# bacpop/sparrowhawk

Hardware: AMD Instinct MI355X
Metric: Gbases/s assembled, k=31 150bp reads (higher is better)
Workload: dtype u64

## Files before the change

### sparrowhawk_amd/csrc/count_part.h

```cpp
#pragma once
#include <hip/hip_runtime.h>
#include <stdint.h>
#include <type_traits>
#include "kmer.h"

namespace shk {

static constexpr int PART_THREADS = 1024;
static constexpr int COUNT_THREADS = 1024;
static constexpr int PART_MAX_P = 16384;

struct PartParams {
    uint32_t P, G, slice_cap;
    int k, m;
    uint32_t max_n;
};

template <int RW> struct Rec { uint64_t w[RW]; };

__device__ __forceinline__ uint64_t sel4(uint32_t b, uint64_t t0, uint64_t t1, uint64_t t2, uint64_t t3) {
    uint64_t lo = (b & 1) ? t1 : t0;
    uint64_t hi = (b & 1) ? t3 : t2;
    return (b & 2) ? hi : lo;
}
// ... 532 lines not shown
    const uint32_t want = 2u * rows;
    return want <= 8u ? 8u : 1u << (32 - __clz((int)(want - 1u)));
}
struct EmitRanges {
    unsigned long long *tab_cursor = nullptr;
    unsigned long long *off = nullptr;
    uint32_t *msk = nullptr, *start = nullptr, *cnt = nullptr, *broken = nullptr;
};

template <int W, typename LT>
__device__ __forceinline__ void table_emit(KmerTable<W> &tb, CountCtlCore &ctl, unsigned long long mine, uint32_t threshold,
                                           unsigned long long *__restrict__ histo, KeyArr<W> out_keys,
                                           uint32_t *__restrict__ out_cnt, unsigned long long out_cap,
                                           unsigned long long *__restrict__ out_cursor, LT *list,
                                           uint32_t *hist_accum = nullptr ,
                                           uint32_t bias = 0 ,
                                           const EmitRanges &er = EmitRanges{}, uint32_t er_g = 0xFFFFFFFFu ) {
    constexpr uint32_t S = KmerTable<W>::S;
    const int lane = threadIdx.x & 63;
    for (int o = 32; o > 0; o >>= 1) mine += __shfl_down(mine, o);
    if (lane == 0 && mine) atomicAdd(&ctl.n_inst, mine);
    for (uint32_t s = threadIdx.x; s < S; s += COUNT_THREADS) {
        uint32_t c = tb.cnt[s];
        if (bias && c) { c = c > 0xFFFFFFFFu - bias ? 0xFFFFFFFFu : c + bias; tb.cnt[s] = c; }
        const unsigned long long m1 = __ballot(c == 1u);
        if (lane == 0 && m1) atomicAdd(&ctl.histo[0], (uint32_t)__popcll(m1));
        if (c > 1u) atomicAdd(&ctl.histo[c >= 500 ? 499 : c - 1], 1u);
        const bool e = c > threshold;
        const unsigned long long em = __ballot(e);
        if (!em) continue;
        uint32_t wb = 0;
        if (lane == 0) wb = atomicAdd(&ctl.n_emit, (uint32_t)__popcll(em));
        wb = __shfl(wb, 0);
        if (e) list[wb + (uint32_t)__popcll(em & ((1ull << lane) - 1ull))] = (LT)s;
    }
    __syncthreads();
    const uint32_t n_emit = ctl.n_emit;
    if (threadIdx.x == 0) {
        unsigned long long base = n_emit ? atomicAdd(out_cursor, (unsigned long long)n_emit) : 0ull;
        if (er.tab_cursor && er_g != 0xFFFFFFFFu) {
            const uint32_t sz = gp_table_size(n_emit);
            const unsigned long long tab_base = atomicAdd(er.tab_cursor, ((unsigned long long)n_emit << 32) | sz);
            er.off[er_g] = (uint32_t)tab_base; er.msk[er_g] = sz - 1u; er.start[er_g] = (uint32_t)base; er.cnt[er_g] = n_emit;
        }
        ctl.emit_base_lo = (uint32_t)base; ctl.emit_base_hi = (uint32_t)(base >> 32);
    }
    if (hist_accum) {
        for (uint32_t b = threadIdx.x; b < 500; b += COUNT_THREADS) hist_accum[b] += ctl.histo[b];
    } else {
        for (uint32_t b = threadIdx.x; b < 500; b += COUNT_THREADS)
            if (ctl.histo[b]) atomicAdd(&histo[b], (unsigned long long)ctl.histo[b]);
    }
    if (!n_emit) return;
    __syncthreads();
    const unsigned long long gbase = ((unsigned long long)ctl.emit_base_hi << 32) | ctl.emit_base_lo;
    for (uint32_t i = threadIdx.x; i < n_emit; i += COUNT_THREADS) {
        const uint32_t sl = list[i];
        const unsigned long long o = gbase + i;
        if (o < out_cap) {
            Kmer<W> x;
            if constexpr (W == 1) x.w[0] = tb.key0[sl];
            else {
#pragma unroll
                for (int j = 0; j < W; j++) x.w[j] = tb.key[j][sl];
            }
            out_keys.store(o, x);
            out_cnt[o] = tb.cnt[sl];
        }
    }
}

struct OvfRec { uint32_t p, est_distinct; unsigned long long instances; };
struct OvfItem { uint32_t p, F, cap, pad; unsigned long long base; };
static constexpr uint32_t OVF_MAX_F = 256;

struct RunView {
    const unsigned long long *run_addr16;
    const uint32_t *run_cnt;
    uint32_t S;
    int k;
    const uint32_t *weights = nullptr;
    unsigned long long rec_base16 = 0;
};

__global__ __launch_bounds__(256) void k_make_runs(const uint32_t *__restrict__ fill, PartParams pp,
                                                   const uint64_t *recs, uint32_t rec_words,
                                                   unsigned long long *__restrict__ run_addr16,
                                                   uint32_t *__restrict__ run_cnt) {
    const uint64_t n = (uint64_t)pp.P * pp.G;
    const unsigned long long base16 = (unsigned long long)recs >> 4;
    for (uint64_t i = (uint64_t)blockIdx.x * blockDim.x + threadIdx.x; i < n; i += (uint64_t)gridDim.x * blockDim.x) {
        run_addr16[i] = base16 + i * pp.slice_cap * (rec_words / 2u);
        run_cnt[i] = min(fill[i], pp.slice_cap);
    }
}

__global__ __launch_bounds__(256) void k_part_totals(const uint32_t *__restrict__ fill, PartParams pp,
                                                     unsigned long long *__restrict__ totals) {
    const uint32_t p = blockIdx.x;
    unsigned long long t = 0;
    for (uint32_t g = threadIdx.x; g < pp.G; g += blockDim.x) t += min(fill[(uint64_t)p * pp.G + g], pp.slice_cap);
    for (int o = 32; o > 0; o >>= 1) t += __shfl_down(t, o);
    __shared__ unsigned long long part[4];
    if ((threadIdx.x & 63) == 0) part[threadIdx.x >> 6] = t;
    __syncthreads();
    if (threadIdx.x == 0) totals[p] = part[0] + part[1] + part[2] + part[3];
}

template <int RW>
__global__ __launch_bounds__(256) void k_pack_partition(const uint64_t *__restrict__ recs,
                                                        const uint32_t *__restrict__ fill, PartParams pp,
                                                        const unsigned long long *__restrict__ base,
                                                        uint64_t *__restrict__ dst) {
    __shared__ uint32_t pre[257];
    const uint32_t p = blockIdx.x;
    const int lane = threadIdx.x & 63;
    if (threadIdx.x < 64) {
        uint32_t run = 0;
        for (uint32_t g0 = 0; g0 < pp.G; g0 += 64) {
            const uint32_t g = g0 + threadIdx.x;
            const uint32_t f = g < pp.G ? min(fill[(uint64_t)p * pp.G + g], pp.slice_cap) : 0u;
            uint32_t incl = f;
            for (int o = 1; o < 64; o <<= 1) { uint32_t v = __shfl_up(incl, o); if (lane >= o) incl += v; }
            if (g < pp.G) pre[g] = run + incl - f;
            run += __shfl(incl, 63);
        }
        if (threadIdx.x == 0) pre[pp.G] = run;
    }
    __syncthreads();
    const uint32_t R = pre[pp.G];
    const uint64_t *src_p = recs + (uint64_t)p * pp.G * pp.slice_cap * RW;
    uint64_t *dst_p = dst + base[p] * RW;
    for (uint32_t r = threadIdx.x; r < R; r += blockDim.x) {
        uint32_t lo = 0, hi = pp.G;
        while (hi - lo > 1) { const uint32_t mid = (lo + hi) >> 1; if (pre[mid] <= r) lo = mid; else hi = mid; }
        const uint64_t *src = src_p + ((uint64_t)lo * pp.slice_cap + (r - pre[lo])) * RW;
#pragma unroll
        for (int o = 0; o < RW; o += 2)
            *reinterpret_cast<ulonglong2 *>(dst_p + (uint64_t)r * RW + o) = *reinterpret_cast<const ulonglong2 *>(src + o);
    }
}

template <int RW>
__global__ __launch_bounds__(256) void k_merge_runs(RunView rvw, const unsigned long long *__restrict__ base,
                                                    uint64_t *__restrict__ dst) {
    __shared__ uint32_t pre[257];
    __shared__ unsigned long long roff[256];
    const uint32_t p = blockIdx.x, S_runs = rvw.S;
    const int lane = threadIdx.x & 63;
    if (threadIdx.x < 64) {
        uint32_t run = 0;
        for (uint32_t g0 = 0; g0 < S_runs; g0 += 64) {
            const uint32_t g = g0 + threadIdx.x;
            const uint32_t f = g < S_runs ? rvw.run_cnt[(uint64_t)p * S_runs + g] : 0u;
            if (g < S_runs) roff[g] = rvw.run_addr16[(uint64_t)p * S_runs + g];
            uint32_t incl = f;
            for (int o = 1; o < 64; o <<= 1) { const uint32_t v = __shfl_up(incl, o); if (lane >= o) incl += v; }
            if (g < S_runs) pre[g] = run + incl - f;
            run += __shfl(incl, 63);
        }
        if (threadIdx.x == 0) pre[S_runs] = run;
    }
    __syncthreads();
    const uint32_t R = pre[S_runs];
    uint64_t *dst_p = dst + base[p] * RW;
    for (uint32_t r = threadIdx.x; r < R; r += blockDim.x) {
        uint32_t lo = 0, hi = S_runs;
        while (hi - lo > 1) { const uint32_t mid = (lo + hi) >> 1; if (pre[mid] <= r) lo = mid; else hi = mid; }
        const uint64_t *src = reinterpret_cast<const uint64_t *>(roff[lo] << 4) + (uint64_t)(r - pre[lo]) * RW;
#pragma unroll
        for (int o = 0; o < RW; o += 2)
            *reinterpret_cast<ulonglong2 *>(dst_p + (uint64_t)r * RW + o) = *reinterpret_cast<const ulonglong2 *>(src + o);
    }
}

template <int W, bool WEIGHTED = false >
__global__ __launch_bounds__(COUNT_THREADS) void k_count_partitions(
    RunView rvw, uint32_t n_parts, uint32_t threshold,
    unsigned long long *__restrict__ histo, KeyArr<W> out_keys, uint32_t *__restrict__ out_cnt,
    unsigned long long out_cap, unsigned long long *__restrict__ out_cursor,
    unsigned long long *__restrict__ n_inst, uint32_t *__restrict__ flags,
    const uint32_t *__restrict__ part_list ,
    OvfRec *__restrict__ ovf ,
    uint32_t *__restrict__ ovf_n,
    uint32_t *__restrict__ work_counter ,
    uint32_t probe_blocks, uint32_t defer_after ) {
    constexpr int RW = 2 * W;
    constexpr uint32_t S = CountShared<W>::S;
    __shared__ CountShared<W> tb;
    __shared__ CountCtl ctl;
    __shared__ uint32_t whist[500];
    __shared__ uint32_t wtot[4];
    const int lane = threadIdx.x & 63;
    const int k = rvw.k;
    const uint32_t S_runs = rvw.S;
    for (uint32_t b = threadIdx.x; b < 500; b += COUNT_THREADS) whist[b] = 0;
    if (threadIdx.x == 0) ctl.n_inst = 0;
    auto load_runs = [&](uint32_t pi, uint32_t &cnt, unsigned long long &addr) {
        cnt = 0; addr = 0;
        if (pi < n_parts && threadIdx.x < S_runs) {
            const uint32_t pp = part_list ? part_list[pi] : pi;
            cnt = rvw.run_cnt[(uint64_t)pp * S_runs + threadIdx.x];
            addr = rvw.run_addr16[(uint64_t)pp * S_runs + threadIdx.x];
        }
    };
    uint32_t nx_cnt; unsigned long long nx_addr;
    load_runs(blockIdx.x, nx_cnt, nx_addr);
  uint32_t pi_next = 0;
  for (uint32_t pi = blockIdx.x; pi < n_parts; pi = pi_next) {
    const uint32_t p = part_list ? part_list[pi] : pi;
    if (threadIdx.x == 0) ctl.next_pi = gridDim.x + atomicAdd(work_counter, 1u);
    {
        const uint32_t f = nx_cnt;
        uint32_t incl = f;
        if (threadIdx.x < 256) {
            for (int o = 1; o < 64; o <<= 1) { const uint32_t v = __shfl_up(incl, o); if (lane >= o) incl += v; }
            if (lane == 63) wtot[threadIdx.x >> 6] = incl;
        }
        __syncthreads();
        if (threadIdx.x < 256) {
            uint32_t off = 0;
            for (uint32_t w = 0; w < (threadIdx.x >> 6); w++) off += wtot[w];
            if (threadIdx.x < S_runs) { ctl.pre[threadIdx.x] = off + incl - f; ctl.roff[threadIdx.x] = nx_addr; }
        }
        if (threadIdx.x == 0) {
            ctl.pre[S_runs] = wtot[0] + wtot[1] + wtot[2] + wtot[3];
            ctl.sp = 1; ctl.st_res[0] = 0; ctl.st_step[0] = 1; ctl.st_factor[0] = 1; ctl.st_next[0] = 0;
            ctl.part_inst = 0; ctl.n_used = 0;
            uint32_t force = 0;
            if (ovf && defer_after && pi >= probe_blocks) {
                const uint32_t x = __hip_atomic_load(&ovf_n[1], __ATOMIC_RELAXED, __HIP_MEMORY_SCOPE_AGENT);
                const uint32_t n_over = x >> 16, n_tried = x & 0xFFFFu;
                force = (n_over >= defer_after && 4u * n_over >= 3u * n_tried) ? 1u : 0u;
            }
            ctl.overflow = force;
        }
    }
    __syncthreads();
    pi_next = ctl.next_pi;
    load_runs(pi_next, nx_cnt, nx_addr);
   [&]() {
    const uint32_t R = ctl.pre[S_runs];
    const bool sat = R >= (1u << 26) || WEIGHTED;

    auto defer = [&](unsigned long long mine, bool was_tried) {
        if (threadIdx.x == 0) ctl.tried = 0;
        __syncthreads();
        for (int o = 32; o > 0; o >>= 1) mine += __shfl_down(mine, o);
        if (lane == 0 && mine) atomicAdd(&ctl.tried, mine);
        unsigned long long inst = 0;
        for (uint32_t r = threadIdx.x; r < R; r += COUNT_THREADS) {
            uint32_t lo = 0, hi = S_runs;
            while (hi - lo > 1) { const uint32_t mid = (lo + hi) >> 1; if (ctl.pre[mid] <= r) lo = mid; else hi = mid; }
            const uint64_t *src = reinterpret_cast<const uint64_t *>(ctl.roff[lo] << 4) + (uint64_t)(r - ctl.pre[lo]) * RW;
            unsigned long long wgt = 1ull;
            if constexpr (WEIGHTED) wgt = rvw.weights[(ctl.roff[lo] - rvw.rec_base16) / W + (r - ctl.pre[lo])];
            inst += ((src[RW - 1] >> 58) + 1ull) * wgt;
        }
        for (int o = 32; o > 0; o >>= 1) inst += __shfl_down(inst, o);
        if (lane == 0 && inst) atomicAdd(&ctl.part_inst, inst);
        __syncthreads();
        if (threadIdx.x == 0 && R) {
            const double est = ctl.tried ? (double)ctl.n_used * (double)ctl.part_inst / (double)ctl.tried : (double)ctl.part_inst;
            const uint32_t slot = atomicAdd(ovf_n, 1u);
            OvfRec o; o.p = p; o.est_distinct = !was_tried ? 0u  : est > 4.0e9 ? 0xFFFFFFFFu : est < 1.0 ? 1u : (uint32_t)est; o.instances = ctl.part_inst;
            ovf[slot] = o;
        }
        if (threadIdx.x == 0 && was_tried && defer_after) atomicAdd(&ovf_n[1], 0x10001u);
    };
    if (ctl.overflow) { defer(0ull, false); return; }

    while (true) {
        __syncthreads();
        if (ctl.sp == 0) break;
        const uint32_t top = ctl.sp - 1;
        const uint32_t res = ctl.st_res[top] + ctl.st_next[top] * ctl.st_step[top], mod = ctl.st_step[top] * ctl.st_factor[top];
        __syncthreads();
        if (threadIdx.x == 0) {
            if (++ctl.st_next[top] == ctl.st_factor[top]) ctl.sp--;
            ctl.n_used = 0; ctl.overflow = 0; ctl.n_emit = 0; ctl.wave_cursor = 0; ctl.rec_used = 0;
            ctl.prog_num = 0; ctl.prog_den = 1;
        }
        table_reset<W>(tb, ctl);

        unsigned long long mine = 0;
        const uint32_t per_wave = (((R + (COUNT_THREADS / 64) - 1) / (COUNT_THREADS / 64)) + 63u) & ~63u;
        const uint32_t w_begin = min(R, (threadIdx.x >> 6) * per_wave), w_end = min(R, w_begin + per_wave);
        uint32_t run_lo = 0, run_next = 0;
        {
            uint32_t lo = 0, hi = S_runs;
            const uint32_t r = min(w_begin + (uint32_t)lane, R ? R - 1u : 0u);
            while (hi - lo > 1) { const uint32_t mid = (lo + hi) >> 1; if (ctl.pre[mid] <= r) lo = mid; else hi = mid; }
            run_lo = lo; run_next = ctl.pre[lo + 1];
        }
        auto fetch = [&](uint32_t r, Rec<RW> &rec, uint32_t &wgt) -> uint32_t {
            wgt = 1u;
            if (r >= w_end) return 0u;
            while (r >= run_next) { run_lo++; run_next = ctl.pre[run_lo + 1]; }
            const uint64_t *src = reinterpret_cast<const uint64_t *>(ctl.roff[run_lo] << 4) + (uint64_t)(r - ctl.pre[run_lo]) * RW;
            if constexpr (WEIGHTED) wgt = rvw.weights[(ctl.roff[run_lo] - rvw.rec_base16) / W + (r - ctl.pre[run_lo])];
#pragma unroll
            for (int o = 0; o < RW; o += 2) {
                const ulonglong2 v2 = *reinterpret_cast<const ulonglong2 *>(src + o);
                rec.w[o] = v2.x; rec.w[o + 1] = v2.y;
            }
            return 1u;
        };
        auto expand = [&](Rec<RW> rec, uint32_t n, uint32_t weight) {
            Kmer<W> f = km_zero<W>();
            for (uint32_t s = 0; s < n; s++) {
                if (ctl.overflow || ctl.n_used > (S / 10) * 9) return;
                if (s) {
#pragma unroll
                    for (int o = 0; o < RW - 1; o++) rec.w[o] = (rec.w[o] >> 2) | (rec.w[o + 1] << 62);
                    rec.w[RW - 1] >>= 2;
                }
                Kmer<W> rv;
#pragma unroll
                for (int j = 0; j < W; j++) rv.w[j] = ~rec.w[j];
                rv.w[W - 1] &= km_topmask<W>(k);
                if (s) km_push_back<W>(f, (uint32_t)(rec.w[W - 1] >> ((2 * (k - 1)) & 63)) & 3u, k);
                else f = km_revcomp<W>(rv, k);
                const bool use_r = km_less<W>(rv, f);
                Kmer<W> c;
#pragma unroll
                for (int j = 0; j < W; j++) c.w[j] = use_r ? rv.w[j] : f.w[j];
                const uint32_t h = km_mix32<W>(c);
                if (mod == 1 || ((h >> 20) & (mod - 1u)) == res) {
                    if (!lds_insert<W>(tb, ctl, c, h ^ __builtin_amdgcn_alignbit(h, h, 19), weight, sat)) ctl.overflow = 1;
                    mine += weight;
                }
            }
        };
        Rec<RW> nxt, nxt2;
#pragma unroll
        for (int o = 0; o < RW; o++) { nxt.w[o] = 0; nxt2.w[o] = 0; }
        uint32_t w_nxt, w_nxt2;
        uint32_t have_nxt = fetch(w_begin + (uint32_t)lane, nxt, w_nxt);
        uint32_t have_nxt2 = fetch(w_begin + 64u + (uint32_t)lane, nxt2, w_nxt2);
        if (threadIdx.x == 0) ctl.prog_den = R ? R : 1u;
        for (uint32_t r0 = w_begin; r0 < w_end; r0 += 64) {
            if (ctl.overflow || ctl.n_used > (S / 10) * 9) { atomicMax(&ctl.prog_num, min(R, (r0 - w_begin) * (COUNT_THREADS / 64) + 1u)); break; }
            Rec<RW> rec = nxt;
            const uint32_t n = have_nxt ? (uint32_t)(rec.w[RW - 1] >> 58) + 1u : 0u;
            if (n) rec_canonicalise<RW>(rec.w, n, k);
            const uint32_t wgt = w_nxt;
            nxt = nxt2; have_nxt = have_nxt2; w_nxt = w_nxt2;
            have_nxt2 = fetch(r0 + 128u + (uint32_t)lane, nxt2, w_nxt2);
            if (n && !rec_insert<W>(tb.rt, ctl, rec, wgt)) {
                if (ovf && mod == 1 && (r0 - w_begin) * 2u < (w_end - w_begin)) ctl.overflow = 1;
                else expand(rec, n, wgt);
            }
        }
        {
            constexpr uint32_t SRc = decltype(tb.rt)::SR;
            auto &rt = tb.rt;
            if (threadIdx.x < 64) rt.nhist[threadIdx.x] = 0;
            __syncthreads();
            for (uint32_t s = threadIdx.x; s < SRc; s += COUNT_THREADS)
                if (rt.rst[s] >= 3u) atomicAdd(&rt.nhist[(uint32_t)(rt.w[s][RW - 1] >> 58)], 1u);
            __syncthreads();
            if (threadIdx.x < 64) {
                const uint32_t v = rt.nhist[threadIdx.x];
                uint32_t incl = v;
                for (int o = 1; o < 64; o <<= 1) { const uint32_t u = __shfl_up(incl, o); if (lane >= o) incl += u; }
                rt.nbase[threadIdx.x] = incl - v;
                if (threadIdx.x == 63) ctl.n_recs = incl;
            }
            __syncthreads();
            for (uint32_t s = threadIdx.x; s < SRc; s += COUNT_THREADS)
                if (rt.rst[s] >= 3u) rt.order[atomicAdd(&rt.nbase[(uint32_t)(rt.w[s][RW - 1] >> 58)], 1u)] = (uint16_t)s;
            __syncthreads();
            const uint32_t n_recs = ctl.n_recs;
            if (threadIdx.x == 0 && ctl.prog_num == 0) ctl.prog_den = n_recs ? n_recs : 1u;
            __syncthreads();
            for (uint32_t i = threadIdx.x; i < n_recs; i += COUNT_THREADS) {
                if (ctl.overflow || ctl.n_used > (S / 10) * 9) { atomicMax(&ctl.prog_num, i - threadIdx.x + 1u); break; }
                const uint32_t s = rt.order[i];
                Rec<RW> rec;
#pragma unroll
                for (int o = 0; o < RW; o++) rec.w[o] = rt.w[s][o];
                expand(rec, (uint32_t)(rec.w[RW - 1] >> 58) + 1u, rt.rst[s] - 2u);
            }
        }
        __syncthreads();
        const bool over = ctl.overflow != 0 || ctl.n_used > (S / 10) * 9;
        if (over && ovf && mod == 1) {
            defer(mine, true);
            return;
        }
        if (over) {
            if (mod >= 4096 || ctl.sp + 1 > 16) { if (threadIdx.x == 0) flags[0] = 1; break; }
            __syncthreads();
            if (threadIdx.x == 0) {
                const uint32_t num = ctl.prog_num ? ctl.prog_num : ctl.prog_den;
                const double est = (double)ctl.n_used * (double)ctl.prog_den / (double)num;
                uint32_t factor = 2;
                while ((double)factor * (0.6 * S) < est && mod * factor < 4096u) factor <<= 1;
                ctl.st_res[ctl.sp] = res; ctl.st_step[ctl.sp] = mod; ctl.st_factor[ctl.sp] = factor; ctl.st_next[ctl.sp] = 0;
                ctl.sp += 1;
            }
            continue;
        }
        static_assert(2u * decltype(tb.rt)::SR >= S, "emit list");
        table_emit<W>(tb, ctl, mine, threshold, histo, out_keys, out_cnt, out_cap, out_cursor, reinterpret_cast<uint16_t *>(tb.rt.rst), whist);
    }
    if (threadIdx.x == 0 && ovf && defer_after) atomicAdd(&ovf_n[1], 1u);
   }();
  }
    __syncthreads();
    for (uint32_t b = threadIdx.x; b < 500; b += COUNT_THREADS)
        if (whist[b]) atomicAdd(&histo[b], (unsigned long long)whist[b]);
    if (threadIdx.x == 0 && ctl.n_inst) atomicAdd(n_inst, ctl.n_inst);
}


template <int W> struct DedupeShared {
    RecTable<W, (W == 1 ? 3072u : ((69632u / (16u * W + 6u)) & ~63u))> rt;
};
template <int W>
__global__ __launch_bounds__(COUNT_THREADS, W <= 2 ? 8 : 4) void k_dedupe_partitions(
                                                                     RunView rvw, uint32_t p_first, uint32_t n_parts,
                                                                     const unsigned long long *__restrict__ base ,
                                                                     unsigned long long base_stride,
                                                                     uint64_t *__restrict__ out_recs, uint32_t *__restrict__ out_w,
                                                                     uint32_t *__restrict__ n_out, uint32_t *__restrict__ work_counter,
                                                                     OvfRec *__restrict__ ovf , uint32_t *__restrict__ ovf_n,
                                                                     uint32_t defer_after, uint32_t kmer_cap,
                                                                     uint32_t *__restrict__ verdict_out ) {
    constexpr int RW = 2 * W;
    __shared__ DedupeShared<W> tb;
    __shared__ CountCtl ctl;
    __shared__ uint32_t wtot[4];
    constexpr uint32_t SR = decltype(tb.rt)::SR;
    const int lane = threadIdx.x & 63;
    const int k = rvw.k;
    const uint32_t S_runs = rvw.S;
    const uint32_t n_here = n_parts - p_first;
    __shared__ uint32_t forced_sh;
    if (threadIdx.x == 0) forced_sh = 0;
    __syncthreads();
    bool forced = false;
    uint32_t pi_next = 0;
    for (uint32_t pi = blockIdx.x; pi < n_here; pi = pi_next) {
        const uint32_t p = p_first + pi;
        uint32_t f = 0; unsigned long long addr = 0;
        if (threadIdx.x < S_runs) { f = rvw.run_cnt[(uint64_t)p * S_runs + threadIdx.x]; addr = rvw.run_addr16[(uint64_t)p * S_runs + threadIdx.x]; }
        forced = forced_sh != 0;
        if (forced) {
            unsigned long long inst = 0;
            const uint64_t *src = reinterpret_cast<const uint64_t *>(addr << 4);
            for (uint32_t i = 0; i < f; i++) inst += (src[(uint64_t)i * RW + RW - 1] >> 58) + 1ull;
            __syncthreads();
            if (threadIdx.x == 0) { ctl.part_inst = 0; ctl.next_pi = gridDim.x + atomicAdd(work_counter, 1u); }
            __syncthreads();
            for (int o = 32; o > 0; o >>= 1) inst += __shfl_down(inst, o);
            if (lane == 0 && inst) atomicAdd(&ctl.part_inst, inst);
            __syncthreads();
            pi_next = ctl.next_pi;
            if (threadIdx.x == 0) {
                n_out[p] = 0;
                if (ctl.part_inst) { const uint32_t slot = atomicAdd(ovf_n, 1u); OvfRec o; o.p = p; o.est_distinct = 0u; o.instances = ctl.part_inst; ovf[slot] = o; }
            }
            continue;
        }
        uint32_t incl = f;
        if (threadIdx.x < 256) {
            for (int o = 1; o < 64; o <<= 1) { const uint32_t v = __shfl_up(incl, o); if (lane >= o) incl += v; }
            if (lane == 63) wtot[threadIdx.x >> 6] = incl;
        }
        __syncthreads();
        if (threadIdx.x < 256) {
            uint32_t off = 0;
            for (uint32_t w = 0; w < (threadIdx.x >> 6); w++) off += wtot[w];
            if (threadIdx.x < S_runs) { ctl.pre[threadIdx.x] = off + incl - f; ctl.roff[threadIdx.x] = addr; }
        }
        if (threadIdx.x == 0) {
            ctl.pre[S_runs] = wtot[0] + wtot[1] + wtot[2] + wtot[3];
            ctl.rec_used = 0; ctl.n_emit = 0; ctl.part_inst = 0;
            ctl.next_pi = gridDim.x + atomicAdd(work_counter, 1u);
        }
        for (uint32_t s = threadIdx.x; s < SR; s += COUNT_THREADS) tb.rt.rst[s] = 0;
        __syncthreads();
        pi_next = ctl.next_pi;
        const uint32_t R = ctl.pre[S_runs];
        auto hand_over = [&]() {
            unsigned long long inst = 0;
            const uint32_t pw = (((R + (COUNT_THREADS / 64) - 1) / (COUNT_THREADS / 64)) + 63u) & ~63u;
            const uint32_t wb = min(R, (threadIdx.x >> 6) * pw), we = min(R, wb + pw);
            uint32_t lo = 0, hi = S_runs;
            { const uint32_t r = min(wb + (uint32_t)lane, R ? R - 1u : 0u);
              while (hi - lo > 1) { const uint32_t mid = (lo + hi) >> 1; if (ctl.pre[mid] <= r) lo = mid; else hi = mid; } }
            uint32_t nx = ctl.pre[lo + 1];
            for (uint32_t r = wb + (uint32_t)lane; r < we; r += 64) {
                while (r >= nx) { lo++; nx = ctl.pre[lo + 1]; }
                const uint64_t *src = reinterpret_cast<const uint64_t *>(ctl.roff[lo] << 4) + (uint64_t)(r - ctl.pre[lo]) * RW;
                inst += (src[RW - 1] >> 58) + 1ull;
            }
            for (int o = 32; o > 0; o >>= 1) inst += __shfl_down(inst, o);
            if (lane == 0 && inst) atomicAdd(&ctl.part_inst, inst);
            __syncthreads();
            if (threadIdx.x == 0) {
                n_out[p] = 0;
                if (R) { const uint32_t slot = atomicAdd(ovf_n, 1u); OvfRec o; o.p = p; o.est_distinct = 0u; o.instances = ctl.part_inst; ovf[slot] = o; }
            }
        };
        const unsigned long long base_p = base ? base[p] : (unsigned long long)p * base_stride;
        uint64_t *dst = out_recs + base_p * RW;
        uint32_t *dst_w = out_w + base_p;
        const uint32_t per_wave = (((R + (COUNT_THREADS / 64) - 1) / (COUNT_THREADS / 64)) + 63u) & ~63u;
        const uint32_t w_begin = min(R, (threadIdx.x >> 6) * per_wave), w_end = min(R, w_begin + per_wave);
        uint32_t run_lo = 0, run_next = 0;
        {
            uint32_t lo = 0, hi = S_runs;
            const uint32_t r = min(w_begin + (uint32_t)lane, R ? R - 1u : 0u);
            while (hi - lo > 1) { const uint32_t mid = (lo + hi) >> 1; if (ctl.pre[mid] <= r) lo = mid; else hi = mid; }
            run_lo = lo; run_next = ctl.pre[lo + 1];
        }
        auto fetch = [&](uint32_t r, Rec<RW> &rec) -> uint32_t {
            if (r >= w_end) return 0u;
            while (r >= run_next) { run_lo++; run_next = ctl.pre[run_lo + 1]; }
            const uint64_t *src = reinterpret_cast<const uint64_t *>(ctl.roff[run_lo] << 4) + (uint64_t)(r - ctl.pre[run_lo]) * RW;
#pragma unroll
            for (int o = 0; o < RW; o += 2) {
                const ulonglong2 v2 = *reinterpret_cast<const ulonglong2 *>(src + o);
                rec.w[o] = v2.x; rec.w[o + 1] = v2.y;
            }
            return 1u;
        };
        Rec<RW> nxt, nxt2;
#pragma unroll
        for (int o = 0; o < RW; o++) { nxt.w[o] = 0; nxt2.w[o] = 0; }
        uint32_t have_nxt = fetch(w_begin + (uint32_t)lane, nxt);
        uint32_t have_nxt2 = fetch(w_begin + 64u + (uint32_t)lane, nxt2);
        for (uint32_t r0 = w_begin; r0 < w_end; r0 += 64) {
            Rec<RW> rec = nxt;
            const uint32_t n = have_nxt ? (uint32_t)(rec.w[RW - 1] >> 58) + 1u : 0u;
            if (n) rec_canonicalise<RW>(rec.w, n, k);
            nxt = nxt2; have_nxt = have_nxt2;
            have_nxt2 = fetch(r0 + 128u + (uint32_t)lane, nxt2);
            const bool pass = n && !rec_insert<W>(tb.rt, ctl, rec);
            const unsigned long long m = __ballot(pass);
            if (m) {
                uint32_t at = 0;
                if (lane == (int)__builtin_ctzll(m)) at = atomicAdd(&ctl.n_emit, (uint32_t)__popcll(m));
                at = __shfl(at, (int)__builtin_ctzll(m)) + (uint32_t)__popcll(m & ((1ull << lane) - 1ull));
                if (pass) { part_store_record<RW>(rec.w, dst + (uint64_t)at * RW); dst_w[at] = 1u; }
            }
        }
        auto &rt = tb.rt;
        if (threadIdx.x < 64) rt.nhist[threadIdx.x] = 0;
        __syncthreads();
        for (uint32_t s = threadIdx.x; s < SR; s += COUNT_THREADS)
            if (rt.rst[s] >= 3u) atomicAdd(&rt.nhist[(uint32_t)(rt.w[s][RW - 1] >> 58)], 1u);
        __syncthreads();
        const uint32_t n_pass = ctl.n_emit;
        if (threadIdx.x < 64) {
            const uint32_t v = rt.nhist[threadIdx.x];
            uint32_t incl2 = v;
            for (int o = 1; o < 64; o <<= 1) { const uint32_t u = __shfl_up(incl2, o); if (lane >= o) incl2 += u; }
            rt.nbase[threadIdx.x] = n_pass + incl2 - v;
            if (threadIdx.x == 63) ctl.n_recs = n_pass + incl2;
        }
        __syncthreads();
        const bool hand = ovf && (ctl.n_recs > kmer_cap || (R > kmer_cap / 4u && 2u * ctl.n_recs > R));
        if (ovf && threadIdx.x == 0 && R) {
            const uint32_t add = hand ? 0x10001u : 1u;
            const uint32_t x = atomicAdd(&ovf_n[1], add) + add;
            const uint32_t n_over = x >> 16, n_tried = x & 0xFFFFu;
            if (defer_after && n_over >= defer_after && 2u * n_over >= n_tried) {
                forced_sh = 1u;
                if (verdict_out) atomicOr(verdict_out, 0x80000000u);
            }
        }
        if (hand) { hand_over(); continue; }
        for (uint32_t s = threadIdx.x; s < SR; s += COUNT_THREADS) {
            const uint32_t st = rt.rst[s];
            if (st < 3u) continue;
            const uint32_t at = atomicAdd(&rt.nbase[(uint32_t)(rt.w[s][RW - 1] >> 58)], 1u);
            uint64_t r[RW];
#pragma unroll
            for (int o = 0; o < RW; o++) r[o] = rt.w[s][o];
            part_store_record<RW>(r, dst + (uint64_t)at * RW);
            dst_w[at] = st - 2u;
        }
        __syncthreads();
        if (threadIdx.x == 0) n_out[p] = ctl.n_recs;
    }
}

template <int W>
__global__ __launch_bounds__(COUNT_THREADS, W <= 2 ? 8 : 4) void k_count_weighted(
    const uint64_t *__restrict__ recs, const uint32_t *__restrict__ weights, const unsigned long long *__restrict__ base ,
    unsigned long long base_stride, const uint32_t *__restrict__ n_recs, uint32_t p_first, uint32_t n_parts, uint32_t merge , int k, uint32_t threshold,
    unsigned long long *__restrict__ histo, KeyArr<W> out_keys, uint32_t *__restrict__ out_cnt,
    unsigned long long out_cap, unsigned long long *__restrict__ out_cursor,
    unsigned long long *__restrict__ n_inst, OvfRec *__restrict__ ovf, uint32_t *__restrict__ ovf_n,
    unsigned long long *__restrict__ work_and_tally ,
    uint32_t probe_groups, uint32_t defer_after,
    EmitRanges er ) {
    constexpr int RW = 2 * W;
    constexpr uint32_t S = KmerTable<W>::S;
    __shared__ KmerTable<W> tb;
    __shared__ CountCtlCore ctl;
    constexpr uint32_t ELIST = W == 1 ? S : 64;
    __shared__ uint16_t elist[ELIST];
    __shared__ uint32_t whist[500];
    __shared__ uint32_t next_g_sh, force_sh;
    const int lane = threadIdx.x & 63;
    for (uint32_t b = threadIdx.x; b < 500; b += COUNT_THREADS) whist[b] = 0;
    if (threadIdx.x == 0) ctl.n_inst = 0;
    const uint32_t n_groups = (n_parts + merge - 1) / merge;
    unsigned long long mine = 0;
    auto count_range = [&](const uint32_t (&pm)[4], uint32_t nm) -> bool {
        uint32_t Rj[4]; unsigned long long bj[4]; uint32_t Rt = 0;
#pragma unroll
        for (int j = 0; j < 4; j++) {
            const bool in = (uint32_t)j < nm;
            Rj[j] = in ? n_recs[pm[j]] : 0u; bj[j] = in ? (base ? base[pm[j]] : (unsigned long long)pm[j] * base_stride) : 0ull;
            Rt += Rj[j];
        }
        auto fetch = [&](uint32_t r, Rec<RW> &rec, uint32_t &wgt) {
            if (r < Rt) {
                unsigned long long at = bj[0] + r;
                uint32_t pre = Rj[0];
#pragma unroll
                for (int j = 1; j < 4; j++) { if (r >= pre) at = bj[j] + (r - pre); pre += Rj[j]; }
                const uint64_t *src = recs + at * RW;
#pragma unroll
                for (int o = 0; o < RW; o += 2) {
// ... 101 lines not shown
        __syncthreads();
        g_next = next_g_sh;
        if (nm == 0) continue;
        if (force_sh) {
#pragma unroll
            for (uint32_t j = 0; j < 4; j++) if (j < nm) defer(pm[j], false);
            continue;
        }
        if (nm > 1 && count_range(pm, nm)) {
            emit(g);
            if (threadIdx.x == 0 && defer_after && in_sample) atomicAdd(tally, nm);
            continue;
        }
        if (nm > 1) mark_broken();
#pragma unroll
        for (uint32_t j = 0; j < 4; j++) {
            if (j >= nm) continue;
            const uint32_t one[4] = {pm[j], 0, 0, 0};
            if (count_range(one, 1u)) { emit(nm == 1 ? g : 0xFFFFFFFFu); if (threadIdx.x == 0 && defer_after && in_sample) atomicAdd(tally, 1u); }
            else defer(pm[j], true);
        }
    }
    __syncthreads();
    for (uint32_t b = threadIdx.x; b < 500; b += COUNT_THREADS)
        if (whist[b]) atomicAdd(&histo[b], (unsigned long long)whist[b]);
    if (threadIdx.x == 0 && ctl.n_inst) atomicAdd(n_inst, ctl.n_inst);
}

template <int RW>
__global__ __launch_bounds__(256) void k_pack_dedup(const uint64_t *__restrict__ src, const uint32_t *__restrict__ src_w,
                                                    const unsigned long long *__restrict__ src_base, const uint32_t *__restrict__ n_out,
                                                    const unsigned long long *__restrict__ dst_base,
                                                    uint64_t *__restrict__ dst, uint32_t *__restrict__ dst_w) {
    const uint32_t p = blockIdx.x, R = n_out[p];
    const uint64_t *sp = src + src_base[p] * RW;
    uint64_t *dp = dst + dst_base[p] * RW;
    for (uint32_t r = threadIdx.x; r < R; r += blockDim.x) {
#pragma unroll
        for (int o = 0; o < RW; o += 2)
            *reinterpret_cast<ulonglong2 *>(dp + (uint64_t)r * RW + o) = *reinterpret_cast<const ulonglong2 *>(sp + (uint64_t)r * RW + o);
        dst_w[dst_base[p] + r] = src_w[src_base[p] + r];
    }
}

static constexpr uint32_t BLOOM_WORDS = 24576;
template <int W, bool BLOOM>
__global__ __launch_bounds__(COUNT_THREADS) void k_ovf_scatter(RunView rvw, const OvfItem *__restrict__ items,
                                                               uint64_t *__restrict__ kmers,
                                                               uint32_t *__restrict__ bucket_fill,
                                                               uint32_t *__restrict__ new_count) {
    constexpr int RW = 2 * W;
    __shared__ uint32_t pre[257];
    __shared__ uint32_t cursor[OVF_MAX_F];
    __shared__ uint32_t bloom[BLOOM ? BLOOM_WORDS : 1];
    __shared__ uint32_t n_new;
    if constexpr (BLOOM) {
        for (uint32_t i = threadIdx.x; i < BLOOM_WORDS; i += COUNT_THREADS) bloom[i] = 0;
        if (threadIdx.x == 0) n_new = 0;
    }
    uint32_t my_new = 0;
    const OvfItem it = items[blockIdx.x];
    const uint32_t p = it.p, S_runs = rvw.S;
    const int lane = threadIdx.x & 63;
    const int k = rvw.k;
    if (threadIdx.x < 64) {
        uint32_t run = 0;
        for (uint32_t g0 = 0; g0 < S_runs; g0 += 64) {
            const uint32_t g = g0 + threadIdx.x;
            uint32_t f = g < S_runs ? rvw.run_cnt[(uint64_t)p * S_runs + g] : 0u;
            uint32_t incl = f;
            for (int o = 1; o < 64; o <<= 1) { uint32_t v = __shfl_up(incl, o); if (lane >= o) incl += v; }
            if (g < S_runs) pre[g] = run + incl - f;
            run += __shfl(incl, 63);
        }
        if (threadIdx.x == 0) pre[S_runs] = run;
    }
    for (uint32_t b = threadIdx.x; b < OVF_MAX_F; b += COUNT_THREADS) cursor[b] = 0;
    __syncthreads();
    const uint32_t R = pre[S_runs];
    const uint32_t F = it.F;
    for (uint32_t r = threadIdx.x; r < R; r += COUNT_THREADS) {
        uint32_t lo = 0, hi = S_runs;
        while (hi - lo > 1) { const uint32_t mid = (lo + hi) >> 1; if (pre[mid] <= r) lo = mid; else hi = mid; }
        const uint64_t *src = reinterpret_cast<const uint64_t *>(rvw.run_addr16[(uint64_t)p * S_runs + lo] << 4) + (uint64_t)(r - pre[lo]) * RW;
        Rec<RW> rec;
#pragma unroll
        for (int o = 0; o < RW; o += 2) {
            const ulonglong2 v2 = *reinterpret_cast<const ulonglong2 *>(src + o);
            rec.w[o] = v2.x; rec.w[o + 1] = v2.y;
        }
        const uint32_t n = (uint32_t)(rec.w[RW - 1] >> 58) + 1u;
        Kmer<W> f = km_zero<W>();
        for (uint32_t s = 0; s < n; s++) {
            if (s) {
#pragma unroll
                for (int o = 0; o < RW - 1; o++) rec.w[o] = (rec.w[o] >> 2) | (rec.w[o + 1] << 62);
                rec.w[RW - 1] >>= 2;
            }
            Kmer<W> rv;
#pragma unroll
            for (int j = 0; j < W; j++) rv.w[j] = ~rec.w[j];
            rv.w[W - 1] &= km_topmask<W>(k);
            if (s) km_push_back<W>(f, (uint32_t)(rec.w[W - 1] >> ((2 * (k - 1)) & 63)) & 3u, k);
            else f = km_revcomp<W>(rv, k);
            const bool use_r = km_less<W>(rv, f);
            Kmer<W> c;
#pragma unroll
            for (int j = 0; j < W; j++) c.w[j] = use_r ? rv.w[j] : f.w[j];
            const uint32_t hk = km_mix32<W>(c);
            if constexpr (BLOOM) {
                const uint32_t h2 = mix32(hk ^ 0xC2B2AE35u);
                const uint32_t word = (uint32_t)(((uint64_t)h2 * BLOOM_WORDS) >> 32);
                const uint32_t b0 = hk & 31u, b1 = (hk >> 5) & 31u;
                const uint32_t bits = (1u << b0) | (1u << (b1 == b0 ? (b0 + 1u) & 31u : b1));
                const uint32_t old = atomicOr(&bloom[word], bits);
                if ((old & bits) != bits) { my_new++; continue; }
            }
            const uint32_t b = (uint32_t)(((uint64_t)mix32(hk ^ 0x85EBCA6Bu) * F) >> 32);
            const uint32_t pos = atomicAdd(&cursor[b], 1u);
            if (pos < it.cap) {
                uint64_t *dst = kmers + (it.base + (unsigned long long)b * it.cap + pos) * W;
#pragma unroll
                for (int j = 0; j < W; j++) dst[j] = c.w[j];
            }
        }
    }
    if constexpr (BLOOM) {
        for (int o = 32; o > 0; o >>= 1) my_new += __shfl_down(my_new, o);
        if (lane == 0 && my_new) atomicAdd(&n_new, my_new);
    }
    __syncthreads();
    for (uint32_t b = threadIdx.x; b < OVF_MAX_F; b += COUNT_THREADS) bucket_fill[(uint64_t)blockIdx.x * OVF_MAX_F + b] = cursor[b];
    if constexpr (BLOOM) { if (threadIdx.x == 0) new_count[blockIdx.x] = n_new; }
}

struct BucketRef { unsigned long long first; uint32_t nb, pad; };

__global__ __launch_bounds__(256) void k_ovf_check(const OvfItem *__restrict__ items, const uint32_t *__restrict__ bucket_fill,
                                                   uint32_t n_items, uint32_t *__restrict__ max_fill,
                                                   BucketRef *__restrict__ list, uint32_t *__restrict__ list_n,
                                                   unsigned long long *__restrict__ sum_fill ) {
    for (uint32_t i = blockIdx.x * blockDim.x + threadIdx.x; i < n_items; i += gridDim.x * blockDim.x) {
        uint32_t mx = 0, ne = 0;
        unsigned long long sm = 0;
        const OvfItem it = items[i];
        for (uint32_t b = 0; b < it.F; b++) {
            const uint32_t f = bucket_fill[(uint64_t)i * OVF_MAX_F + b];
            mx = max(mx, f); ne += f != 0; sm += f;
        }
        max_fill[i] = mx; sum_fill[i] = sm;
        if (mx > it.cap || !ne) continue;
        uint32_t at = atomicAdd(list_n, ne);
        for (uint32_t b = 0; b < it.F; b++) {
            const uint32_t f = bucket_fill[(uint64_t)i * OVF_MAX_F + b];
            if (f) { BucketRef r; r.first = it.base + (unsigned long long)b * it.cap; r.nb = f; r.pad = 0; list[at++] = r; }
        }
    }
}

template <int W>
__global__ __launch_bounds__(COUNT_THREADS, 8) void k_count_buckets(
    const BucketRef *__restrict__ list, uint32_t n_list, const uint64_t *__restrict__ kmers,
    uint32_t threshold, unsigned long long *__restrict__ histo, KeyArr<W> out_keys, uint32_t *__restrict__ out_cnt,
    unsigned long long out_cap, unsigned long long *__restrict__ out_cursor,
    unsigned long long *__restrict__ n_inst, uint32_t *__restrict__ flags,
    uint32_t bias , unsigned long long *__restrict__ n_keys ) {
    constexpr uint32_t S = KmerTable<W>::S;
    constexpr int PF = (int)((S * 114u / 100u + COUNT_THREADS - 1) / COUNT_THREADS);
    constexpr uint32_t PF_MAX = (uint32_t)PF * COUNT_THREADS;
    __shared__ KmerTable<W> tb;
    __shared__ CountCtlCore ctl;
// ... 140 lines not shown
```

Before: 174.2.

## Rotate triple record buffers and use global address space loads in counting loops

Run record loads now go through explicitly global-address-space pointers, so the compiler can emit global loads instead of flat ones. The counting loops replace the copy-based two-deep prefetch with a rotating three-buffer scheme unrolled by three, and fetches clamp the index instead of branching. Loop bounds are made wave-uniform with readfirstlane. The W>1 path drops to a one-deep prefetch, and an explicit vmem wait after each emit store may add stalls.

```diff
diff --git a/sparrowhawk_amd/csrc/count_part.h b/sparrowhawk_amd/csrc/count_part.h
--- a/sparrowhawk_amd/csrc/count_part.h
+++ b/sparrowhawk_amd/csrc/count_part.h
@@ -638,6 +638,15 @@
     const uint32_t *weights = nullptr;
     unsigned long long rec_base16 = 0;
 };
+__device__ __forceinline__ const SHK_GLOBAL uint64_t *run_recs(unsigned long long a16) {
+    return reinterpret_cast<const SHK_GLOBAL uint64_t *>(a16 << 4);
+}
+__device__ __forceinline__ void vmem_wait_all() { __builtin_amdgcn_s_waitcnt(0x0F70); }
+typedef unsigned long long shk_u64x2 __attribute__((ext_vector_type(2)));
+__device__ __forceinline__ ulonglong2 run_load16(const SHK_GLOBAL uint64_t *src, int o) {
+    const shk_u64x2 v = *reinterpret_cast<const SHK_GLOBAL shk_u64x2 *>(src + o);
+    return make_ulonglong2(v.x, v.y);
+}
 
 __global__ __launch_bounds__(256) void k_make_runs(const uint32_t *__restrict__ fill, PartParams pp,
                                                    const uint64_t *recs, uint32_t rec_words,
@@ -723,10 +732,10 @@
     for (uint32_t r = threadIdx.x; r < R; r += blockDim.x) {
         uint32_t lo = 0, hi = S_runs;
         while (hi - lo > 1) { const uint32_t mid = (lo + hi) >> 1; if (pre[mid] <= r) lo = mid; else hi = mid; }
-        const uint64_t *src = reinterpret_cast<const uint64_t *>(roff[lo] << 4) + (uint64_t)(r - pre[lo]) * RW;
+        const SHK_GLOBAL uint64_t *src = run_recs(roff[lo]) + (uint64_t)(r - pre[lo]) * RW;
 #pragma unroll
         for (int o = 0; o < RW; o += 2)
-            *reinterpret_cast<ulonglong2 *>(dst_p + (uint64_t)r * RW + o) = *reinterpret_cast<const ulonglong2 *>(src + o);
+            *reinterpret_cast<ulonglong2 *>(dst_p + (uint64_t)r * RW + o) = run_load16(src, o);
     }
 }
 
@@ -808,7 +817,7 @@
         for (uint32_t r = threadIdx.x; r < R; r += COUNT_THREADS) {
             uint32_t lo = 0, hi = S_runs;
             while (hi - lo > 1) { const uint32_t mid = (lo + hi) >> 1; if (ctl.pre[mid] <= r) lo = mid; else hi = mid; }
-            const uint64_t *src = reinterpret_cast<const uint64_t *>(ctl.roff[lo] << 4) + (uint64_t)(r - ctl.pre[lo]) * RW;
+            const SHK_GLOBAL uint64_t *src = run_recs(ctl.roff[lo]) + (uint64_t)(r - ctl.pre[lo]) * RW;
             unsigned long long wgt = 1ull;
             if constexpr (WEIGHTED) wgt = rvw.weights[(ctl.roff[lo] - rvw.rec_base16) / W + (r - ctl.pre[lo])];
             inst += ((src[RW - 1] >> 58) + 1ull) * wgt;
@@ -840,8 +849,9 @@
         table_reset<W>(tb, ctl);
 
         unsigned long long mine = 0;
-        const uint32_t per_wave = (((R + (COUNT_THREADS / 64) - 1) / (COUNT_THREADS / 64)) + 63u) & ~63u;
-        const uint32_t w_begin = min(R, (threadIdx.x >> 6) * per_wave), w_end = min(R, w_begin + per_wave);
+        const uint32_t R_u = __builtin_amdgcn_readfirstlane(R);
+        const uint32_t per_wave = (((R_u + (COUNT_THREADS / 64) - 1) / (COUNT_THREADS / 64)) + 63u) & ~63u;
+        const uint32_t w_begin = min(R_u, (uint32_t)__builtin_amdgcn_readfirstlane(threadIdx.x >> 6) * per_wave), w_end = min(R_u, w_begin + per_wave);
         uint32_t run_lo = 0, run_next = 0;
         {
             uint32_t lo = 0, hi = S_runs;
@@ -849,18 +859,16 @@
             while (hi - lo > 1) { const uint32_t mid = (lo + hi) >> 1; if (ctl.pre[mid] <= r) lo = mid; else hi = mid; }
             run_lo = lo; run_next = ctl.pre[lo + 1];
         }
-        auto fetch = [&](uint32_t r, Rec<RW> &rec, uint32_t &wgt) -> uint32_t {
-            wgt = 1u;
-            if (r >= w_end) return 0u;
+        auto fetch = [&](uint32_t r0, Rec<RW> &rec, uint32_t &wgt) {
+            const uint32_t r = min(r0 + (uint32_t)lane, w_end - 1u);
             while (r >= run_next) { run_lo++; run_next = ctl.pre[run_lo + 1]; }
-            const uint64_t *src = reinterpret_cast<const uint64_t *>(ctl.roff[run_lo] << 4) + (uint64_t)(r - ctl.pre[run_lo]) * RW;
+            const SHK_GLOBAL uint64_t *src = run_recs(ctl.roff[run_lo]) + (uint64_t)(r - ctl.pre[run_lo]) * RW;
             if constexpr (WEIGHTED) wgt = rvw.weights[(ctl.roff[run_lo] - rvw.rec_base16) / W + (r - ctl.pre[run_lo])];
 #pragma unroll
             for (int o = 0; o < RW; o += 2) {
-                const ulonglong2 v2 = *reinterpret_cast<const ulonglong2 *>(src + o);
+                const ulonglong2 v2 = run_load16(src, o);
                 rec.w[o] = v2.x; rec.w[o + 1] = v2.y;
             }
-            return 1u;
         };
         auto expand = [&](Rec<RW> rec, uint32_t n, uint32_t weight) {
             Kmer<W> f = km_zero<W>();
@@ -888,25 +896,34 @@
                 }
             }
         };
-        Rec<RW> nxt, nxt2;
-#pragma unroll
-        for (int o = 0; o < RW; o++) { nxt.w[o] = 0; nxt2.w[o] = 0; }
-        uint32_t w_nxt, w_nxt2;
-        uint32_t have_nxt = fetch(w_begin + (uint32_t)lane, nxt, w_nxt);
-        uint32_t have_nxt2 = fetch(w_begin + 64u + (uint32_t)lane, nxt2, w_nxt2);
-        if (threadIdx.x == 0) ctl.prog_den = R ? R : 1u;
-        for (uint32_t r0 = w_begin; r0 < w_end; r0 += 64) {
-            if (ctl.overflow || ctl.n_used > (S / 10) * 9) { atomicMax(&ctl.prog_num, min(R, (r0 - w_begin) * (COUNT_THREADS / 64) + 1u)); break; }
-            Rec<RW> rec = nxt;
-            const uint32_t n = have_nxt ? (uint32_t)(rec.w[RW - 1] >> 58) + 1u : 0u;
+        uint32_t stopped = 0;
+        auto batch = [&](uint32_t r0, Rec<RW> &rec, const uint32_t &wgt_in, Rec<RW> &ahead, uint32_t &w_ahead) {
+            if (!stopped && r0 < w_end && __builtin_amdgcn_readfirstlane((uint32_t)(ctl.overflow || ctl.n_used > (S / 10) * 9))) {
+                atomicMax(&ctl.prog_num, min(R, (r0 - w_begin) * (COUNT_THREADS / 64) + 1u));
+                stopped = 1;
+            }
+            const uint32_t n = !stopped && r0 + (uint32_t)lane < w_end ? (uint32_t)(rec.w[RW - 1] >> 58) + 1u : 0u;
             if (n) rec_canonicalise<RW>(rec.w, n, k);
-            const uint32_t wgt = w_nxt;
-            nxt = nxt2; have_nxt = have_nxt2; w_nxt = w_nxt2;
-            have_nxt2 = fetch(r0 + 128u + (uint32_t)lane, nxt2, w_nxt2);
+            const uint32_t wgt = wgt_in;
+            fetch(r0 + 128u, ahead, w_ahead);
             if (n && !rec_insert<W>(tb.rt, ctl, rec, wgt)) {
                 if (ovf && mod == 1 && (r0 - w_begin) * 2u < (w_end - w_begin)) ctl.overflow = 1;
                 else expand(rec, n, wgt);
             }
+        };
+        if (threadIdx.x == 0) ctl.prog_den = R ? R : 1u;
+        if (w_begin < w_end) {
+            Rec<RW> buf_a, buf_b, buf_c;
+            uint32_t w_a = 1u, w_b = 1u, w_c = 1u;
+            fetch(w_begin, buf_a, w_a);
+            fetch(w_begin + 64u, buf_b, w_b);
+            uint32_t r0 = w_begin;
+            do {
+                batch(r0, buf_a, w_a, buf_c, w_c);
+                batch(r0 + 64u, buf_b, w_b, buf_a, w_a);
+                batch(r0 + 128u, buf_c, w_c, buf_b, w_b);
+                r0 += 192u;
+            } while (r0 < w_end && !stopped);
         }
         {
             constexpr uint32_t SRc = decltype(tb.rt)::SR;
@@ -1005,7 +1022,7 @@
         forced = forced_sh != 0;
         if (forced) {
             unsigned long long inst = 0;
-            const uint64_t *src = reinterpret_cast<const uint64_t *>(addr << 4);
+            const SHK_GLOBAL uint64_t *src = run_recs(addr);
             for (uint32_t i = 0; i < f; i++) inst += (src[(uint64_t)i * RW + RW - 1] >> 58) + 1ull;
             __syncthreads();
             if (threadIdx.x == 0) { ctl.part_inst = 0; ctl.next_pi = gridDim.x + atomicAdd(work_counter, 1u); }
@@ -1050,7 +1067,7 @@
             uint32_t nx = ctl.pre[lo + 1];
             for (uint32_t r = wb + (uint32_t)lane; r < we; r += 64) {
                 while (r >= nx) { lo++; nx = ctl.pre[lo + 1]; }
-                const uint64_t *src = reinterpret_cast<const uint64_t *>(ctl.roff[lo] << 4) + (uint64_t)(r - ctl.pre[lo]) * RW;
+                const SHK_GLOBAL uint64_t *src = run_recs(ctl.roff[lo]) + (uint64_t)(r - ctl.pre[lo]) * RW;
                 inst += (src[RW - 1] >> 58) + 1ull;
             }
             for (int o = 32; o > 0; o >>= 1) inst += __shfl_down(inst, o);
@@ -1064,8 +1081,9 @@
         const unsigned long long base_p = base ? base[p] : (unsigned long long)p * base_stride;
         uint64_t *dst = out_recs + base_p * RW;
         uint32_t *dst_w = out_w + base_p;
-        const uint32_t per_wave = (((R + (COUNT_THREADS / 64) - 1) / (COUNT_THREADS / 64)) + 63u) & ~63u;
-        const uint32_t w_begin = min(R, (threadIdx.x >> 6) * per_wave), w_end = min(R, w_begin + per_wave);
+        const uint32_t R_u = __builtin_amdgcn_readfirstlane(R);
+        const uint32_t per_wave = (((R_u + (COUNT_THREADS / 64) - 1) / (COUNT_THREADS / 64)) + 63u) & ~63u;
+        const uint32_t w_begin = min(R_u, (uint32_t)__builtin_amdgcn_readfirstlane(threadIdx.x >> 6) * per_wave), w_end = min(R_u, w_begin + per_wave);
         uint32_t run_lo = 0, run_next = 0;
         {
             uint32_t lo = 0, hi = S_runs;
@@ -1073,28 +1091,20 @@
             while (hi - lo > 1) { const uint32_t mid = (lo + hi) >> 1; if (ctl.pre[mid] <= r) lo = mid; else hi = mid; }
             run_lo = lo; run_next = ctl.pre[lo + 1];
         }
-        auto fetch = [&](uint32_t r, Rec<RW> &rec) -> uint32_t {
-            if (r >= w_end) return 0u;
+        auto fetch = [&](uint32_t r0, Rec<RW> &rec) {
+            const uint32_t r = min(r0 + (uint32_t)lane, w_end - 1u);
             while (r >= run_next) { run_lo++; run_next = ctl.pre[run_lo + 1]; }
-            const uint64_t *src = reinterpret_cast<const uint64_t *>(ctl.roff[run_lo] << 4) + (uint64_t)(r - ctl.pre[run_lo]) * RW;
+            const SHK_GLOBAL uint64_t *src = run_recs(ctl.roff[run_lo]) + (uint64_t)(r - ctl.pre[run_lo]) * RW;
 #pragma unroll
             for (int o = 0; o < RW; o += 2) {
-                const ulonglong2 v2 = *reinterpret_cast<const ulonglong2 *>(src + o);
+                const ulonglong2 v2 = run_load16(src, o);
                 rec.w[o] = v2.x; rec.w[o + 1] = v2.y;
             }
-            return 1u;
         };
-        Rec<RW> nxt, nxt2;
-#pragma unroll
-        for (int o = 0; o < RW; o++) { nxt.w[o] = 0; nxt2.w[o] = 0; }
-        uint32_t have_nxt = fetch(w_begin + (uint32_t)lane, nxt);
-        uint32_t have_nxt2 = fetch(w_begin + 64u + (uint32_t)lane, nxt2);
-        for (uint32_t r0 = w_begin; r0 < w_end; r0 += 64) {
-            Rec<RW> rec = nxt;
-            const uint32_t n = have_nxt ? (uint32_t)(rec.w[RW - 1] >> 58) + 1u : 0u;
+        auto batch = [&](uint32_t r0, Rec<RW> &rec, Rec<RW> &ahead) {
+            const uint32_t n = r0 + (uint32_t)lane < w_end ? (uint32_t)(rec.w[RW - 1] >> 58) + 1u : 0u;
             if (n) rec_canonicalise<RW>(rec.w, n, k);
-            nxt = nxt2; have_nxt = have_nxt2;
-            have_nxt2 = fetch(r0 + 128u + (uint32_t)lane, nxt2);
+            fetch(r0 + (W == 1 ? 128u : 64u), ahead);
             const bool pass = n && !rec_insert<W>(tb.rt, ctl, rec);
             const unsigned long long m = __ballot(pass);
             if (m) {
@@ -1102,6 +1112,28 @@
                 if (lane == (int)__builtin_ctzll(m)) at = atomicAdd(&ctl.n_emit, (uint32_t)__popcll(m));
                 at = __shfl(at, (int)__builtin_ctzll(m)) + (uint32_t)__popcll(m & ((1ull << lane) - 1ull));
                 if (pass) { part_store_record<RW>(rec.w, dst + (uint64_t)at * RW); dst_w[at] = 1u; }
+                vmem_wait_all();
+            }
+        };
+        if constexpr (W == 1) {
+          if (w_begin < w_end) {
+            Rec<RW> buf_a, buf_b, buf_c;
+            fetch(w_begin, buf_a);
+            fetch(w_begin + 64u, buf_b);
+            uint32_t r0 = w_begin;
+            do {
+                batch(r0, buf_a, buf_c);
+                batch(r0 + 64u, buf_b, buf_a);
+                batch(r0 + 128u, buf_c, buf_b);
+                r0 += 192u;
+            } while (r0 < w_end);
+          }
+        } else {
+            Rec<RW> nxt;
+            if (w_begin < w_end) fetch(w_begin, nxt);
+            for (uint32_t r0 = w_begin; r0 < w_end; r0 += 64) {
+                Rec<RW> rec = nxt;
+                batch(r0, rec, nxt);
             }
         }
         auto &rt = tb.rt;
@@ -1369,11 +1401,11 @@
     for (uint32_t r = threadIdx.x; r < R; r += COUNT_THREADS) {
         uint32_t lo = 0, hi = S_runs;
         while (hi - lo > 1) { const uint32_t mid = (lo + hi) >> 1; if (pre[mid] <= r) lo = mid; else hi = mid; }
-        const uint64_t *src = reinterpret_cast<const uint64_t *>(rvw.run_addr16[(uint64_t)p * S_runs + lo] << 4) + (uint64_t)(r - pre[lo]) * RW;
+        const SHK_GLOBAL uint64_t *src = run_recs(rvw.run_addr16[(uint64_t)p * S_runs + lo]) + (uint64_t)(r - pre[lo]) * RW;
         Rec<RW> rec;
 #pragma unroll
         for (int o = 0; o < RW; o += 2) {
-            const ulonglong2 v2 = *reinterpret_cast<const ulonglong2 *>(src + o);
+            const ulonglong2 v2 = run_load16(src, o);
             rec.w[o] = v2.x; rec.w[o + 1] = v2.y;
         }
         const uint32_t n = (uint32_t)(rec.w[RW - 1] >> 58) + 1u;
```

Measured after the change: 170.6. -2.1%, worse.
